# rwdavies/QUILT

Hardware: AMD Instinct MI355X
Metric: samples/sec on 2Mb region, K=50k haps, 1x coverage; dosage r2 vs CPU ref (higher is better)
Workload: dtype f64

## Files before the change

quilt_amd/csrc/gibbs.hip:

```cpp
#include "panel.hpp"

#include <chrono>
#include <functional>

#include <algorithm>
#include <cmath>
#include <cstdlib>
#include <map>
#include <memory>

#include "gibbs_dev.hpp"
#include "gibbs_blocks.hpp"

namespace qa {
int gibbs3_waves(int Ksp, int C, int share);
void launch_gibbs3(const void *gibbs_params, hipStream_t st);
void launch_block_rate3(const void *gibbs_params, hipStream_t st);
void launch_block3(const void *gibbs_params, hipStream_t st);
void launch_resample3(const void *gibbs_params, hipStream_t st);
}

namespace {

template <int NE, int NW>
__device__ void forward_full_both(Chain<NE, NW> &ch) {
    const int G = ch.G, Ksp = ch.Ksp;
    Col<NE> a[2], e[2];
    GridStreams<Chain<NE, NW>> gs;
    for (int g = 0; g < G; g++) {
        if ((g & 63) == 0) {
            if (g) gs.store_c(ch);
            gs.load_fwd(ch, g);
        }
        const int j = g & 63;
        ch.ld(e[0], ch.eg[0] + (size_t)g * Ksp);
        ch.ld(e[1], ch.eg[1] + (size_t)g * Ksp);
        const double s0 = rl_f64(gs.t0, j), s1 = rl_f64(gs.t1, j);
#pragma unroll
        for (int h = 0; h < 2; h++) {
#pragma unroll
            for (int i = 0; i < NE; i++) {
                if (g == 0) a[h].v[i] = ch.valid[i] ? ch.prior * e[h].v[i] : 0.0;
                else a[h].v[i] = ch.valid[i] ? e[h].v[i] * (s0 * a[h].v[i] + s1 * ch.prior) : 0.0;
            }
        }
        double sm[2];
        ch.sum_col2(a[0], a[1], sm[0], sm[1]);
        const double cc[2] = {1 / sm[0], 1 / sm[1]};
#pragma unroll
        for (int h = 0; h < 2; h++) {
#pragma unroll
            for (int i = 0; i < NE; i++) a[h].v[i] = a[h].v[i] * cc[h];
            ch.st(a[h], ch.alpha[h] + (size_t)g * Ksp);
        }
        gs.set_c(ch.lane, j, cc[0], cc[1]);
    }
    gs.store_c(ch);
    chain_sync<NW>();
}

template <int NE, int NW, bool FASTER>
__device__ void backward_both(Chain<NE, NW> &ch) {
    const int G = ch.G, Ksp = ch.Ksp;
    const double one_over_K = 1 / (double)ch.Ks;
    Col<NE> b[2], e[2];
    GridStreams<Chain<NE, NW>> gs;
    gs.load_bwd(ch, (G - 1) & ~63);
    {
        const int j = (G - 1) & 63;
        const double cl[2] = {rl_f64(gs.c0, j), rl_f64(gs.c1, j)};
#pragma unroll
        for (int h = 0; h < 2; h++) {
#pragma unroll
            for (int i = 0; i < NE; i++) b[h].v[i] = ch.valid[i] ? cl[h] : 0.0;
            ch.stm(b[h], ch.beta[h] + (size_t)(G - 1) * Ksp);
        }
    }
    if (G >= 2) {
        ch.ldm(e[0], ch.eg[0] + (size_t)(G - 1) * Ksp);
        ch.ldm(e[1], ch.eg[1] + (size_t)(G - 1) * Ksp);
    }
    for (int g = G - 2; g >= 0; --g) {
        if ((g & 63) == 63) gs.load_bwd(ch, g & ~63);
        const int j = g & 63;
        Col<NE> en[2];
        ch.ldm(en[0], ch.eg[0] + (size_t)g * Ksp);
        ch.ldm(en[1], ch.eg[1] + (size_t)g * Ksp);
        const double s0 = rl_f64(gs.t0, j), s1 = rl_f64(gs.t1, j);
        const double cg[2] = {rl_f64(gs.c0, j), rl_f64(gs.c1, j)};
        const bool has = !FASTER || rl_i32(gs.has, j) != 0;
        double x[2] = {0, 0};
#pragma unroll
        for (int h = 0; h < 2; h++) {
#pragma unroll
            for (int i = 0; i < NE; i++) {
                if (has) b[h].v[i] = e[h].v[i] * b[h].v[i];
                if (FASTER) x[h] += b[h].v[i];
                else x[h] += ch.valid[i] ? ch.prior * b[h].v[i] : 0.0;
            }
        }
        ch.template bsum<2>(x);
#pragma unroll
        for (int h = 0; h < 2; h++) {
            const double xx = FASTER ? s1 * x[h] * one_over_K : s1 * x[h];
#pragma unroll
            for (int i = 0; i < NE; i++) b[h].v[i] = ch.valid[i] ? cg[h] * (xx + s0 * b[h].v[i]) : 0.0;
            ch.stm(b[h], ch.beta[h] + (size_t)g * Ksp);
        }
        e[0] = en[0];
        e[1] = en[1];
    }
}

#ifndef QA_LEAN_WAVES
#define QA_LEAN_WAVES 2
#endif
template <int NE, int NW, bool LEAN>
__global__ __launch_bounds__(64 * NW) __attribute__((amdgpu_waves_per_eu(LEAN ? QA_LEAN_WAVES : 1))) void k_gibbs(GibbsParams p) {
    __shared__ double s_red[2 * NW * 4];
    __shared__ double s_e[LEAN ? 2 * NE * 64 * NW : 1];
    const int c = blockIdx.x, t = threadIdx.x;
    using CH = Chain<NE, NW>;
    CH ch(p, c, t, s_red);
    constexpr int NT = CH::NT;
    const int lane = ch.lane;
    const int G = ch.G, Ksp = ch.Ksp, R = ch.R, Ks = ch.Ks;
    const double prior = ch.prior;
    bool (&valid)[NE] = ch.valid;
    const double *runif = p.seed_reads ? nullptr : p.runif_reads + (size_t)p.read_off[c] * p.n_its;
    const uint64_t seed_reads = p.seed_reads ? p.seed_reads[c] : 0, seed_shard = p.seed_shard ? p.seed_shard[c] : 0;
    const int first_read = p.first_read[c];
    const bool init_iteratively = p.init_iteratively && first_read >= 0;

    for (int h = 0; h < 3; h++)
        for (int g = t; g < G; g += NT) ch.cv[h][g] = 0.0;
    for (int r = t; r < R; r += NT) ch.Hc[r] = 0;

    {
        Col<NE> one;
#pragma unroll
        for (int i = 0; i < NE; i++) one.v[i] = 1.0;
        for (int h = 0; h < 2; h++)
            for (int g = 0; g < G; g++) ch.st(one, ch.eg[h] + (size_t)g * Ksp);
    }
    chain_sync<NW>();
    if (!init_iteratively) {
        ReadStreams<CH> rs;
        rs.base = -1;
        int r = 0;
        while (r < R) {
            if ((r & 63) == 0 && rs.base != r) rs.load(ch, r, nullptr, 0);
            const int g = rl_i32(rs.wif, r & 63);
            Col<NE> e[2];
#pragma unroll
            for (int i = 0; i < NE; i++) e[0].v[i] = e[1].v[i] = 1.0;
            while (r < R) {
                if ((r & 63) == 0 && rs.base != r) rs.load(ch, r, nullptr, 0);
                if (rl_i32(rs.wif, r & 63) != g) break;
                Col<NE> er;
                {
                    typename CH::ErPre x;
                    ch.ld_pre(x, r);
                    ch.read_emission(er, x, rl_i32(rs.dn, r & 63));
                }
                const int h = rl_i32(rs.H, r & 63) - 1;
#pragma unroll
                for (int i = 0; i < NE; i++) {
                    if (h == 0) e[0].v[i] *= er.v[i];
                    else e[1].v[i] *= er.v[i];
                }
                r++;
            }
            ch.st(e[0], ch.eg[0] + (size_t)g * Ksp);
            ch.st(e[1], ch.eg[1] + (size_t)g * Ksp);
        }
        forward_full_both(ch);
        backward_both<NE, NW, false>(ch);
    } else {
        Col<NE> one;
#pragma unroll
        for (int i = 0; i < NE; i++) one.v[i] = valid[i] ? 1.0 : 0.0;
        for (int h = 0; h < 2; h++) {
            for (int g = 0; g < G; g++) {
                ch.st(one, ch.alpha[h] + (size_t)g * Ksp);
                ch.st(one, ch.beta[h] + (size_t)g * Ksp);
            }
            for (int g = t; g < G; g += NT) ch.cv[h][g] = 1.0;
        }
        chain_sync<NW>();
        for (int h = 0; h < 2; h++) {
            Col<NE> a;
#pragma unroll
            for (int i = 0; i < NE; i++) a.v[i] = valid[i] ? prior * 1.0 : 0.0;
            const double cc = 1 / ch.sum_col(a);
#pragma unroll
            for (int i = 0; i < NE; i++) a.v[i] = a.v[i] * cc;
            ch.st(a, ch.alpha[h]);
            if (t == 0) ch.cv[h][0] = cc;
        }
    }
    chain_sync<NW>();

    int shard_it = 0;
    int status = 0;
    for (int it = 0; it < p.n_its && status == 0; it++) {
        const bool last_sweep = it == p.n_its - 1;
        const bool steady = !init_iteratively || it >= 2;
        Col<NE> a[2];
        int iRead = 0;
        typename CH::ErPre pre_er;
        if (R > 0) ch.ld_pre(pre_er, 0);
        ReadStreams<CH> rs;
        rs.base = -1;
        GridStreams<CH> gs;
        Col<NE> e[2], bt[2];
        ch.ldm(e[0], ch.eg[0]);
        ch.ldm(e[1], ch.eg[1]);
        ch.ldm(bt[0], ch.beta[0]);
        ch.ldm(bt[1], ch.beta[1]);
        for (int g = 0; g < G; g++) {
            if ((g & 63) == 0) {
                if (g) gs.store_c(ch);
                gs.load_fwd(ch, g);
            }
            const int jg = g & 63;
            const bool has = rl_i32(gs.has, jg) != 0;
            Col<NE> en[LEAN ? 1 : 2], bn[LEAN ? 1 : 2];
            if constexpr (!LEAN) {
                const size_t gn = (size_t)min(g + 1, G - 1) * Ksp;
                ch.ldm(en[0], ch.eg[0] + gn);
                ch.ldm(en[1], ch.eg[1] + gn);
                ch.ldm(bn[0], ch.beta[0] + gn);
                ch.ldm(bn[1], ch.beta[1] + gn);
            }
            double cg[2];
            if (g > 0) {
                const double x = rl_f64(gs.t0, jg), t1 = rl_f64(gs.t1, jg);
                const double one_over_K = 1 / (double)Ks;
                const double c2v[2] = {rl_f64(gs.c0, jg), rl_f64(gs.c1, jg)};
                double sp[2];
                ch.sum_col2(a[0], a[1], sp[0], sp[1]);
#pragma unroll
                for (int h = 0; h < 2; h++) {
                    const double alphaConst = t1 * sp[h];
#pragma unroll
                    for (int i = 0; i < NE; i++) {
                        const double inner = (x * a[h].v[i] + alphaConst * one_over_K);
                        a[h].v[i] = valid[i] ? (has ? e[h].v[i] * inner : inner) : 0.0;
                    }
                }
                double sn[2];
                ch.sum_col2(a[0], a[1], sn[0], sn[1]);
#pragma unroll
                for (int h = 0; h < 2; h++) {
                    const double c2 = c2v[h];
                    double aa = 1 / (c2 * sn[h]);
                    cg[h] = c2 * aa;
                    aa *= c2;
#pragma unroll
                    for (int i = 0; i < NE; i++) a[h].v[i] *= aa;
                }
            } else {
#pragma unroll
                for (int h = 0; h < 2; h++) {
#pragma unroll
                    for (int i = 0; i < NE; i++) a[h].v[i] = valid[i] ? prior * e[h].v[i] : 0.0;
                }
                double sn[2];
                ch.sum_col2(a[0], a[1], sn[0], sn[1]);
#pragma unroll
                for (int h = 0; h < 2; h++) {
                    cg[h] = 1 / sn[h];
#pragma unroll
                    for (int i = 0; i < NE; i++) a[h].v[i] *= cg[h];
                }
            }
            bool changed = false;
            Col<NE> ab[2];
            double pC[2] = {1, 1};
            if (has) {
                double s[2] = {0, 0};
#pragma unroll
                for (int i = 0; i < NE; i++) {
                    ab[0].v[i] = a[0].v[i] * bt[0].v[i];
                    ab[1].v[i] = a[1].v[i] * bt[1].v[i];
                    s[0] += ab[0].v[i];
                    s[1] += ab[1].v[i];
                }
                ch.template bsum<2>(s);
// ... 85 lines not shown
                const double cs0 = p0, cs1 = p1 + p0;
                const int h_rN = (chance < cs0) ? 0 : ((chance < cs1) ? 1 : 0);
                if (((h_rN != h_rC) || ginit) && !pass) {
                    changed = true;
                    if (lane == jr) rs.H = h_rN + 1;
                    auto mul_e = [&](int h, const Col<NE> &f) {
                        if constexpr (LEAN) {
#pragma unroll
                            for (int i = 0; i < NE; i++) s_e[(h * NE + i) * NT + t] *= f.v[i];
                        } else {
#pragma unroll
                            for (int i = 0; i < NE; i++) e[h].v[i] *= f.v[i];
                        }
                    };
                    if (normal) {
                        if (h_rC == 0) {
#pragma unroll
                            for (int i = 0; i < NE; i++) { a[0].v[i] *= ri.v[i]; ab[0].v[i] *= ri.v[i]; }
                            mul_e(0, ri);
                        } else {
#pragma unroll
                            for (int i = 0; i < NE; i++) { a[1].v[i] *= ri.v[i]; ab[1].v[i] *= ri.v[i]; }
                            mul_e(1, ri);
                        }
                    }
                    if (h_rN == 0) {
#pragma unroll
                        for (int i = 0; i < NE; i++) { a[0].v[i] *= er.v[i]; ab[0].v[i] *= er.v[i]; }
                        mul_e(0, er);
                    } else {
#pragma unroll
                        for (int i = 0; i < NE; i++) { a[1].v[i] *= er.v[i]; ab[1].v[i] *= er.v[i]; }
                        mul_e(1, er);
                    }
                    if (normal || h_rN == 1) { pC[0] = pA1[0]; pC[1] = pA1[1]; }
                }
                if (last_sweep) {
                    const double x[3] = {p0, p1, 0.0};
                    const double rlc[7][3] = {{1, 0, 0}, {0, 1, 0}, {0, 0, 1}, {0.5 / (0.5 + 0.5), 0.5 / (0.5 + 0.5), 0},
                                              {0.5 / (0.5 + 0.0), 0, 0.0 / (0.5 + 0.0)},
                                              {0, 0.5 / (0.5 + 0.0), 0.0 / (0.5 + 0.0)}, {0.5, 0.5, 0.0}};
                    double local_min = 2;
                    int which = 8;
                    for (int i = 0; i < 7; i++) {
                        const double y = fabs(rlc[i][0] - x[0]) + fabs(rlc[i][1] - x[1]) + fabs(rlc[i][2] - x[2]);
                        if (y < local_min) { local_min = y; which = i; }
                    }
                    if (lane == jr) rs.Hc = (local_min < p.class_sum_cutoff) ? which + 1 : 0;
                }
            }
#ifndef QA_LEAN_LATE_E
            if constexpr (LEAN) {
                const size_t gn0 = (size_t)min(g + 1, G - 1) * Ksp;
                ch.ldm(e[0], ch.eg[0] + gn0);
                ch.ldm(e[1], ch.eg[1] + gn0);
            }
#endif
            if (changed) {
                double sm[2];
                ch.sum_col2(a[0], a[1], sm[0], sm[1]);
#pragma unroll
                for (int h = 0; h < 2; h++) {
                    const double alphaConst = 1 / sm[h];
                    cg[h] *= alphaConst;
#pragma unroll
                    for (int i = 0; i < NE; i++) a[h].v[i] = a[h].v[i] * alphaConst;
#ifndef QA_LEAN_LATE_E
                    if constexpr (LEAN) {
#pragma unroll
                        for (int i = 0; i < NE; i++) bt[h].v[i] = s_e[(h * NE + i) * NT + t];
                        ch.stm(bt[h], ch.eg[h] + (size_t)g * Ksp);
                    } else {
                        ch.stm(e[h], ch.eg[h] + (size_t)g * Ksp);
                    }
#else
                    if constexpr (LEAN) {
#pragma unroll
                        for (int i = 0; i < NE; i++) e[h].v[i] = s_e[(h * NE + i) * NT + t];
                    }
                    ch.stm(e[h], ch.eg[h] + (size_t)g * Ksp);
#endif
                }
            }
            if (last_sweep) {
#pragma unroll
                for (int h = 0; h < 2; h++) ch.stm(a[h], ch.alpha[h] + (size_t)g * Ksp);
            }
            gs.set_c(lane, jg, cg[0], cg[1]);
            if constexpr (LEAN) {
#ifndef QA_DBG_NO_LATE_LOADS
                const size_t gn = (size_t)min(g + 1, G - 1) * Ksp;
#ifdef QA_LEAN_LATE_E
                ch.ldm(e[0], ch.eg[0] + gn);
                ch.ldm(e[1], ch.eg[1] + gn);
#endif
                ch.ldm(bt[0], ch.beta[0] + gn);
                ch.ldm(bt[1], ch.beta[1] + gn);
#endif
            } else {
                e[0] = en[0]; e[1] = en[1];
                bt[0] = bn[0]; bt[1] = bn[1];
            }
        }
        gs.store_c(ch);
        if (rs.base >= 0) rs.store(ch);
        chain_sync<NW>();
#ifndef QA_DBG_SKIP_BWD
        backward_both<NE, NW, true>(ch);
#endif
        {
            double s[2] = {0, 0};
            for (int g = t; g < G; g += NT) { s[0] += ch.cv[0][g]; s[1] += ch.cv[1][g]; }
            ch.template bsum<2>(s);
            if (!isfinite(s[0]) || !isfinite(s[1])) status = 1;
        }
        if (p.per_it) {
            double s[4] = {0, 0, 0, 0};
            for (int g = t; g < G; g += NT) { s[0] -= log(ch.cv[0][g]); s[1] -= log(ch.cv[1][g]); }
            for (int r = t; r < R; r += NT) { const int h = ch.H[r]; s[2] += h == 1 ? 1.0 : 0.0; s[3] += h == 2 ? 1.0 : 0.0; }
            ch.template bsum<4>(s);
            if (t == 0) {
                double *o = p.per_it + ((size_t)c * p.n_its + it) * 8;
                o[0] = s[0]; o[1] = s[1]; o[2] = 0; o[3] = s[2]; o[4] = s[3]; o[5] = 0; o[6] = 0; o[7] = 0;
            }
        }
        if (status) break;
        bool to_block = false;
        for (int i = 0; i < p.n_block; i++) if (p.block_its[i] == it) to_block = true;
#ifdef QA_DBG_SKIP_SHARD
        to_block = false;
#endif
        if (to_block && p.do_shard) {
            const double *ru = p.runif_shard + ((size_t)c * p.n_block + shard_it) * (G - 1);
            shard_it++;
            double mloc1, mloc2, mlc1 = 0, mlc2 = 0;
            {
                double s[2] = {0, 0};
                for (int g = t; g < G; g += NT) { s[0] -= log(ch.cv[0][g]); s[1] -= log(ch.cv[1][g]); }
                ch.template bsum<2>(s);
                mloc1 = s[0]; mloc2 = s[1];
            }
            bool flip = false;
            int ir = 0;
            Col<NE> s_a[2];
            GridStreams<CH> ss;
            ReadStreams<CH> rr;
            rr.base = -1;
            bool rr_dirty = false;
            for (int g = 0; g < G; g++) {
                if ((g & 63) == 0) {
                    if (g) ss.store_c(ch);
                    ss.load_fwd(ch, g);
                }
                const int jg = g & 63;
                const double oc1 = rl_f64(ss.c0, jg), oc2 = rl_f64(ss.c1, jg);
                Col<NE> e2[2];
                ch.ldm(e2[0], ch.eg[flip ? 1 : 0] + (size_t)g * Ksp);
                ch.ldm(e2[1], ch.eg[flip ? 0 : 1] + (size_t)g * Ksp);
                Col<NE> b1, b2;
                if (!LEAN && g < G - 1) {
                    ch.ldm(b1, ch.beta[0] + (size_t)g * Ksp);
                    ch.ldm(b2, ch.beta[1] + (size_t)g * Ksp);
                }
                double cn[2];
                if (g == 0) {
#pragma unroll
                    for (int h = 0; h < 2; h++) {
#pragma unroll
                        for (int i = 0; i < NE; i++) s_a[h].v[i] = valid[i] ? prior * e2[h].v[i] : 0.0;
                    }
                    double sm[2];
                    ch.sum_col2(s_a[0], s_a[1], sm[0], sm[1]);
#pragma unroll
                    for (int h = 0; h < 2; h++) {
                        cn[h] = 1 / sm[h];
#pragma unroll
                        for (int i = 0; i < NE; i++) s_a[h].v[i] *= cn[h];
                    }
                } else {
                    if (flip) {
                        ch.stm(e2[0], ch.eg[0] + (size_t)g * Ksp);
                        ch.stm(e2[1], ch.eg[1] + (size_t)g * Ksp);
                    }
                    const double x = rl_f64(ss.t0, jg), t1 = rl_f64(ss.t1, jg);
                    double sp[2];
                    ch.sum_col2(s_a[0], s_a[1], sp[0], sp[1]);
#pragma unroll
                    for (int h = 0; h < 2; h++) {
                        const double alphaConst = t1 * sp[h];
                        const double c2 = (h == 0) ? oc1 : oc2;
#pragma unroll
                        for (int i = 0; i < NE; i++)
                            s_a[h].v[i] = valid[i] ? c2 * e2[h].v[i] * (x * s_a[h].v[i] + alphaConst * prior) : 0.0;
                    }
                    double sm[2];
                    ch.sum_col2(s_a[0], s_a[1], sm[0], sm[1]);
#pragma unroll
                    for (int h = 0; h < 2; h++) {
                        const double c2 = (h == 0) ? oc1 : oc2;
                        const double aa = 1 / sm[h];
                        cn[h] = c2 * aa;
#pragma unroll
                        for (int i = 0; i < NE; i++) s_a[h].v[i] *= aa;
                    }
                }
                if (last_sweep) {
                    ch.stm(s_a[0], ch.alpha[0] + (size_t)g * Ksp);
                    ch.stm(s_a[1], ch.alpha[1] + (size_t)g * Ksp);
                }
                ss.set_c(lane, jg, cn[0], cn[1]);
                mlc1 -= log(cn[0]);
                mlc2 -= log(cn[1]);
                while (ir < R) {
                    if ((ir & 63) == 0 && rr.base != ir) {
                        if (rr.base >= 0 && rr_dirty) rr.store(ch);
                        rr.load(ch, ir, nullptr, 0);
                        rr_dirty = false;
                    }
                    if (rl_i32(rr.wif, ir & 63) != g) break;
                    if (flip) {
                        if (lane == (ir & 63)) rr.H = 3 - rr.H;
                        rr_dirty = true;
                    }
                    ir++;
                }
                if (g < G - 1) {
                    if constexpr (LEAN) {
                        ch.ldm(b1, ch.beta[0] + (size_t)g * Ksp);
                        ch.ldm(b2, ch.beta[1] + (size_t)g * Ksp);
                    }
                    double s[4] = {0, 0, 0, 0};
#pragma unroll
                    for (int i = 0; i < NE; i++) {
                        s[0] += s_a[0].v[i] * b1.v[i];
                        s[1] += s_a[1].v[i] * b2.v[i];
                        s[2] += s_a[1].v[i] * b1.v[i];
                        s[3] += s_a[0].v[i] * b2.v[i];
                    }
                    ch.template bsum<4>(s);
                    const double pA1 = mlc1 + mloc1 + log(s[0]);
                    const double pA2 = mlc2 + mloc2 + log(s[1]);
                    const double pB1 = mlc2 + mloc1 + log(s[2]);
                    const double pB2 = mlc1 + mloc2 + log(s[3]);
                    const double diff = pB1 + pB2 - pA1 - pA2;
                    double probs1 = 1;
                    const double probs2 = exp(diff);
                    const double ps = probs1 + probs2;
                    probs1 /= ps;
                    const double ug = seed_shard ? stream_uniform(seed_shard, (uint64_t)(shard_it - 1) * (G - 1) + g) : ru[g];
                    flip = ug > probs1;
                }
                mloc1 += log(oc1);
                mloc2 += log(oc2);
            }
            ss.store_c(ch);
            if (rr.base >= 0 && rr_dirty) rr.store(ch);
            chain_sync<NW>();
            backward_both<NE, NW, false>(ch);
        }
    }
    if (t == 0) p.status[c] = status;
}

__global__ __launch_bounds__(256) void k_happrobs(GibbsParams p) {
    const int g = blockIdx.x, c = blockIdx.y;
    const int b = threadIdx.x & 31, part = threadIdx.x >> 5;
    __shared__ double s_g[3][8][32], s_t[3][8];
    extern __shared__ __attribute__((aligned(16))) char s_dyn[];
    const int Ks = p.Ks, Ksp = p.Ksp, G = p.G;
    double *const s_gk0 = reinterpret_cast<double *>(s_dyn);
    uint32_t *const s_w = reinterpret_cast<uint32_t *>(s_gk0 + (size_t)p.nH * Ksp);
    auto gk = [&](int h, int k) -> double & { return s_gk0[(size_t)h * Ksp + k]; };
    const int32_t *which = p.which + (size_t)c * Ks;
    const size_t mat = (size_t)G * Ksp;
    for (int k = threadIdx.x; k < Ks; k += 256) {
        const int kk = which[k];
        s_w[k] = panel_word(p, g, kk, p.hm[(size_t)g * p.Kp + kk]);
        for (int h = 0; h < p.nH; h++) {
            const size_t o = ((size_t)c * p.nH + h) * mat + (size_t)g * Ksp + k;
            const double x = 1 / p.cvec[((size_t)c * 3 + h) * G + g];
            gk(h, k) = (p.alpha[o] * p.beta[o]) * x;
        }
    }
    __syncthreads();
    const int s = 32 * g, nLocal = min(32, p.T - s);
    double acc[3] = {0, 0, 0}, tot[3] = {0, 0, 0};
    if (p.nH == 2) {
        for (int k = part; k < Ks; k += 8) {
            const bool on = (s_w[k] >> b) & 1u;
// ... 394 lines not shown
    GibbsLaunch(GibbsLaunch &&) = default;
    GibbsLaunch(const GibbsLaunch &) = delete;
};

GibbsLaunch launch_slice(const GibbsCall &a, const qa_gibbs_opts_t *o, const std::vector<size_t> &base_of, int G, int T, int c0, int c1) {
    GibbsLaunch L;
    L.c0 = c0; L.C = c1 - c0;
    const size_t chain0 = (size_t)c0, read0 = (size_t)a.read_off[c0], base0 = base_of[chain0];
    const size_t n_its = (size_t)(o->n_gibbs_burn_in_its + o->n_gibbs_sample_its), nb = (size_t)o->n_block_gibbs_iterations;
    auto from = [](auto *p, size_t off) { return p ? p + off : nullptr; };
    L.ff_chain = from(o->ff_chain, chain0);
    L.rep_id = from(o->reads_same_as, chain0);
    L.a.which = a.which + chain0 * o->Ks;
    L.a.first_read = a.first_read + chain0;
    L.a.underflow_problem = from(a.underflow_problem, chain0);
    L.a.seed_reads = from(a.seed_reads, chain0);
    L.a.seed_shard = from(a.seed_shard, chain0);
    L.a.hapProbs_t = from(a.hapProbs_t, chain0 * T * 3);
    L.a.genProbsM_t = from(a.genProbsM_t, chain0 * T * 3);
    L.a.genProbsF_t = from(a.genProbsF_t, chain0 * T * 3);
    L.a.state_out = a.state_out;
    L.read_off.resize((size_t)L.C + 1);
    for (int i = 0; i <= L.C; i++) L.read_off[(size_t)i] = a.read_off[c0 + i] - a.read_off[c0];
    L.a.read_off = L.read_off.data();
    L.a.read_ptr = a.read_ptr + read0 + chain0;
    L.a.wif = a.wif + read0;
    L.a.H = a.H + read0;
    L.a.H_class = from(a.H_class, read0);
    L.a.runif_reads = from(a.runif_reads, read0 * n_its);
    L.a.runif_shard = from(a.runif_shard, o->ff != 0.0 ? read0 * nb * 2 : chain0 * nb * (size_t)(G - 1));
    L.a.u = a.u + base0;
    L.a.bq = a.bq + base0;
    if (o->reads_same_as) {
        L.rep_off.resize((size_t)L.C);
        for (int c = c0; c < c1; c++) L.rep_off[(size_t)(c - c0)] = (int64_t)base_of[(size_t)o->reads_same_as[c]] - (int64_t)base0;
    }
    return L;
}

inline int32_t fold_base_quality(int32_t b, int32_t &last) {
    if (b == 0) b = last; else last = b;
    if (b > 255 || b < -255) throw std::runtime_error("|base quality| > 255");
    return b;
}

void fold_zero_base_qualities(const int32_t *rp, int R, int Jmax, int32_t *bq_eff_block) {
    int32_t last = 0;
    for (int r = 0; r < R; r++) {
        int J = rp[r + 1] - rp[r] - 1;
        if (J >= Jmax) J = Jmax;
        for (int j = 0; j <= J; j++) bq_eff_block[rp[r] + j] = fold_base_quality(bq_eff_block[rp[r] + j], last);
    }
}

std::vector<int32_t> checked_folded_qualities(int n, const int32_t *read_off, const int32_t *read_ptr, const int32_t *u, const int32_t *bq,
                                              const std::vector<int32_t> &base_off, int T, int Jmax) {
    std::vector<int32_t> bq_eff((size_t)std::max(base_off[n], 1));
    qa::parallel_for((size_t)n, qa::host_threads(), [&](size_t c) {
        const int R = read_off[c + 1] - read_off[c];
        const int32_t *rp = read_ptr + read_off[c] + c;
        const size_t b0 = (size_t)base_off[c];
        for (int i = 0; i < rp[R]; i++) {
            if (u[b0 + i] < 0 || u[b0 + i] >= T) throw std::runtime_error("read SNP index out of range");
            bq_eff[b0 + i] = bq[b0 + i];
        }
        fold_zero_base_qualities(rp, R, Jmax, bq_eff.data() + b0);
    });
    return bq_eff;
}

struct ChunkHost {
    int C, G, T, Ks, Ksp, NE, nH, n_its, nw, er_nt, er_padb, rc_words, totR, totB, maxR = 0;
    bool want_probs, want_pairs;
    bool aliased = false;
    size_t etot = 0, ixtot = 0;
    std::vector<int32_t> base_off, which0, bq_eff, dense_of, n_dense;
    std::vector<size_t> eoff, ixoff;
    std::vector<uint8_t> ghr;
    std::vector<uint32_t> rc_any;
    std::vector<int32_t> rep;
    std::vector<int64_t> hbase;
};

ChunkHost chunk_layout(qa_panel_t *pn, const qa_rare_common *rc, const qa_gibbs_opts_t *o, const GibbsLaunch &L) {
    ChunkHost h;
    const int C = h.C = L.C;
    h.G = rc ? rc->G_all : pn->G; h.T = rc ? rc->T_all : pn->T; h.Ks = o->Ks;
    h.Ksp = (h.Ks + 63) / 64 * 64; h.NE = h.Ksp / 64;
    h.nH = o->ff != 0.0 ? 3 : 2;
    h.rc_words = rc ? (h.T + 31) / 32 : 0;
    h.n_its = o->n_gibbs_burn_in_its + o->n_gibbs_sample_its;
    h.totR = L.a.read_off[C];
    h.want_probs = wants_probs(L.a, o);
    h.want_pairs = rc && h.want_probs && h.Ks <= 1024;
    h.nw = o->ff != 0.0 ? qa::gibbs3_waves(h.Ksp, C, pn->sharers()) : choose_gibbs_waves(h.Ksp, C, pn->exclusive ? 0 : pn->share);
    h.er_nt = 64 * h.nw; h.er_padb = padb_of(h.NE / h.nw);
    h.rc_any.assign((size_t)C * h.rc_words, 0u);
    h.base_off.assign(C + 1, 0); h.which0.resize((size_t)C * h.Ks);
    h.eoff.resize(C); h.ixoff.resize(C);
    h.ghr.assign((size_t)C * h.G, 0);
    h.dense_of.assign(std::max(h.totR, 1), -1);
    h.n_dense.assign(C, 0);
    for (int c = 0; c < C; c++) {
        const int R = L.a.read_off[c + 1] - L.a.read_off[c];
        h.maxR = std::max(h.maxR, R);
        const int32_t *rp = L.a.read_ptr + L.a.read_off[c] + c;
        h.base_off[c + 1] = h.base_off[c] + rp[R];
        h.ixoff[c] = h.ixtot;
        h.ixtot += (size_t)R * h.er_nt * h.er_padb;
    }
    h.totB = h.base_off[C];
    h.bq_eff.resize((size_t)std::max(h.totB, 1));
    return h;
}

void find_shared_reads(const GibbsLaunch &L, ChunkHost &h) {
    const int32_t *read_off = L.a.read_off, *read_ptr = L.a.read_ptr;
    const auto &base_off = h.base_off;
    h.rep.resize(h.C); h.hbase.resize(h.C);
    std::map<int32_t, int32_t> first_of;
    for (int c = 0; c < h.C; c++) {
        h.rep[c] = c;
        h.hbase[c] = L.rep_id ? L.rep_off[c] : (int64_t)base_off[c];
        if (!L.rep_id) continue;
        auto it = first_of.find(L.rep_id[c]);
        if (it == first_of.end()) { first_of.emplace(L.rep_id[c], c); h.aliased |= L.rep_off[c] != (int64_t)base_off[c]; continue; }
        const int r0 = it->second;
        const int R = read_off[c + 1] - read_off[c];
        if (read_off[r0 + 1] - read_off[r0] != R || base_off[r0 + 1] - base_off[r0] != base_off[c + 1] - base_off[c] ||
            std::memcmp(read_ptr + read_off[r0] + r0, read_ptr + read_off[c] + c, sizeof(int32_t) * ((size_t)R + 1)) != 0)
            throw std::runtime_error("reads_same_as names a chain with other reads");
        h.rep[c] = r0;
        h.aliased = true;
    }
}

void prepare_chain(const qa_panel_t *pn, const qa_rare_common *rc, const qa_gibbs_opts_t *o, const GibbsLaunch &L, ChunkHost &h, int c) {
    const int32_t *read_off = L.a.read_off, *wif = L.a.wif;
    const int G = h.G, T = h.T, Ks = h.Ks, rc_words = h.rc_words;
    const bool is_rep = h.rep[c] == c;
    const int R = read_off[c + 1] - read_off[c];
    const int32_t *rp = L.a.read_ptr + read_off[c] + c;
    const int64_t hb = h.hbase[c];
    int32_t *bq_eff = h.bq_eff.data() + (size_t)h.base_off[h.rep[c]];
    if (is_rep) std::memcpy(bq_eff, L.a.bq + hb, sizeof(int32_t) * (size_t)(h.base_off[c + 1] - h.base_off[c]));
    for (int r = 0; r < R; r++) {
        const int g = wif[read_off[c] + r];
        if (g < 0 || g >= G) throw std::runtime_error("read grid index out of range");
        if (r > 0 && g < wif[read_off[c] + r - 1]) throw std::runtime_error("reads must be sorted by grid");
        h.ghr[(size_t)c * G + g] = 1;
    }
    for (int k = 0; k < Ks; k++) {
        const int v = L.a.which[(size_t)c * Ks + k] - 1;
        if (v < 0 || v >= pn->K) throw std::runtime_error("which_haps_to_use out of range");
        h.which0[(size_t)c * Ks + k] = v;
        if (rc)
            for (int64_t i = rc->h_rare_ptr[v]; i < rc->h_rare_ptr[v + 1]; i++) {
                const int t = rc->h_rare_snp[i];
                h.rc_any[(size_t)c * rc_words + (t >> 5)] |= 1u << (t & 31);
            }
    }
    const int32_t *cu = L.a.u + hb;
    int32_t last = 0;
    int nd = 0;
    for (int r = 0; r < R; r++) {
        int J = rp[r + 1] - rp[r] - 1;
// ... 95 lines not shown
}

void upload_rare_pairs(qa::GibbsScratch &S, const qa_rare_common *rc, const ChunkHost &h, hipStream_t st) {
    const int C = h.C, G = h.G, Ks = h.Ks;
    std::vector<size_t> pbase((size_t)C + 1, 0);
    std::vector<std::vector<uint32_t>> keys((size_t)C);
    qa::parallel_for((size_t)C, qa::host_threads(), [&](size_t c) {
        auto &kv = keys[c];
        for (int k = 0; k < Ks; k++) {
            const int v = h.which0[c * Ks + k];
            for (int64_t i = rc->h_rare_ptr[v]; i < rc->h_rare_ptr[v + 1]; i++) kv.push_back(((uint32_t)rc->h_rare_snp[i] << 10) | (uint32_t)k);
        }
        std::sort(kv.begin(), kv.end());
    });
    for (int c = 0; c < C; c++) pbase[(size_t)c + 1] = pbase[(size_t)c] + keys[(size_t)c].size();
    std::vector<uint16_t> pairs(std::max<size_t>(pbase[(size_t)C], 1));
    std::vector<int32_t> poff((size_t)C * (G + 1), 0);
    for (int c = 0; c < C; c++) {
        const auto &kv = keys[(size_t)c];
        int32_t *po = poff.data() + (size_t)c * (G + 1);
        size_t i = 0;
        for (int g = 0; g < G; g++) {
            po[g] = (int32_t)i;
            while (i < kv.size() && (int)((kv[i] >> 10) >> 5) == g) {
                pairs[pbase[(size_t)c] + i] = (uint16_t)((((kv[i] >> 10) & 31u) << 10) | (kv[i] & 1023u));
                i++;
            }
        }
        po[G] = (int32_t)i;
    }
    S.rc_pairs.ensure(pairs.size()); S.rc_pairs.upload(pairs.data(), pairs.size(), st);
    S.rc_pair_off.ensure(poff.size()); S.rc_pair_off.upload(poff.data(), poff.size(), st);
    S.rc_pair_base.ensure((size_t)C); S.rc_pair_base.upload(pbase.data(), (size_t)C, st);
}

void carve_arena(qa::GibbsScratch &S, qa::Arena &arena, size_t arena_need, const ChunkHost &h) {
    const size_t mat = (size_t)h.C * h.nH * h.G * h.Ksp;
    S.er_idx.arena = S.er_tab.arena = &arena;
    S.eMatRead.arena = S.alpha.arena = S.beta.arena = S.eg.arena = S.cvec.arena = S.hap.arena = S.gm.arena = S.gf.arena = &arena;
    arena.require(arena_need);
    arena.reset();
    S.eMatRead.ensure(std::max<size_t>(h.etot, 1));
    S.er_idx.ensure(std::max<size_t>(h.ixtot, 1));
    S.er_tab.ensure(std::max<size_t>((size_t)h.totR * 64, 1));
    S.alpha.ensure(mat); S.beta.ensure(mat); S.eg.ensure(mat);
    S.cvec.ensure((size_t)h.C * 3 * h.G);
    if (h.want_probs) {
        S.hap.ensure((size_t)h.C * h.T * 3); S.gm.ensure((size_t)h.C * h.T * 3); S.gf.ensure((size_t)h.C * h.T * 3);
    }
}

GibbsParams fill_params(const qa::GibbsScratch &S, const qa_panel_t *pn, const qa_rare_common *rc, const qa_gibbs_opts_t *o,
                        const GibbsLaunch &L, const ChunkHost &h, hipStream_t st) {
    const int C = h.C;
    GibbsParams prm{};
    prm.hm = pn->hm.p; prm.B = pn->B.p; prm.sp_off = pn->sp_off.p; prm.sp_k = pn->sp_k.p;
    prm.sp_word = pn->sp_word.p; prm.sigma = S.tm.p; prm.Kp = pn->Kp; prm.G = h.G; prm.T = h.T;
    prm.nMaxDH = pn->nMaxDH; prm.ref_error = pn->ref_error;
    prm.C = C; prm.Ks = h.Ks; prm.Ksp = h.Ksp; prm.NE = h.NE; prm.which = S.which.p;
    prm.read_off = S.read_off.p; prm.read_ptr = S.read_ptr.p; prm.base_off = S.base_off.p;
    prm.u = S.u.p; prm.bq = S.bq.p; prm.wif = S.wif.p; prm.grid_has_read = S.ghr.p;
    prm.pR_tab = S.tabs.p; prm.pA_tab = S.tabs.p + 512;
    prm.Jmax = o->Jmax; prm.inv_maxdiff = 1 / o->maxDifferenceBetweenReads; prm.rescale = o->rescale_eMatRead_t;
    prm.n_its = h.n_its; prm.n_burn_in = o->n_gibbs_burn_in_its; prm.block_its = S.block_its.p;
    prm.n_block = o->perform_block_gibbs ? o->n_block_gibbs_iterations : 0;
    prm.do_shard = o->do_shard_block_gibbs; prm.init_iteratively = o->gibbs_initialize_iteratively;
    prm.disable_read_category_usage = o->disable_read_category_usage;
    prm.class_sum_cutoff = o->class_sum_cutoff;
    prm.nH = h.nH;
    prm.it_begin = 0; prm.it_end = h.n_its;
    prm.ff = o->ff;
    if (o->per_it_out) {
        QA_HIP(hipMemsetAsync(S.per_it.p, 0, sizeof(double) * C * h.n_its * 8, st));
        prm.per_it = S.per_it.p;
    }
    if (L.ff_chain) prm.ff_chain = S.ff_chain.p;
    prm.runif_reads = S.runif_reads.p; prm.first_read = S.first_read.p; prm.runif_shard = S.runif_shard.p;
    prm.seed_reads = L.a.seed_reads ? S.seeds.p : nullptr;
    prm.seed_shard = (L.a.seed_reads && L.a.seed_shard) ? S.seeds.p + C : nullptr;
    prm.eMatRead = S.eMatRead.p; prm.eread_off = S.eread_off.p; prm.is_cat1 = S.is_cat1.p; prm.er_nent = S.er_nent.p;
    prm.er_idx = S.er_idx.p; prm.eridx_off = S.eridx_off.p; prm.er_tab = S.er_tab.p; prm.dense_of = S.dense_of.p;
    prm.er_nt = h.er_nt; prm.er_padb = h.er_padb;
    prm.alpha = S.alpha.p; prm.beta = S.beta.p; prm.eg = S.eg.p; prm.cvec = S.cvec.p;
    prm.H = S.H.p; prm.H_class = S.H_class.p; prm.status = S.status.p;
    prm.hapProbs = S.hap.p; prm.genProbsM = S.gm.p; prm.genProbsF = S.gf.p;
    if (rc) {
        prm.rc_common = rc->common_index.p; prm.rc_rare_ptr = rc->rare_ptr.p; prm.rc_rare_snp = rc->rare_snp.p;
        prm.rc_any = S.rc_any.p; prm.rc_words = h.rc_words; prm.rc_Gc = pn->G;
        if (h.want_pairs) { prm.rc_pairs = S.rc_pairs.p; prm.rc_pair_off = S.rc_pair_off.p; prm.rc_pair_base = S.rc_pair_base.p; }
    }
    return prm;
}

void nipt_block_tables(const qa_gibbs_opts_t *o, const GibbsLaunch &L, const ChunkHost &h, const std::vector<double> &rate2,
                       const std::vector<int32_t> &seg_status, int n_thr, std::vector<int32_t> &h_where, std::vector<int32_t> &h_tab,
                       std::vector<int32_t> &h_n) {
    const int C = h.C, G = h.G;
    const int32_t *read_off = L.a.read_off;
    h_where.assign((size_t)C * G, -1); h_tab.assign((size_t)C * 4 * G, 0); h_n.assign(C, 0);
    qa::parallel_for((size_t)C, n_thr, [&](size_t c) {
        const int R = read_off[c + 1] - read_off[c];
        if (seg_status[c] != 0 || R < 1) return;
        const std::vector<int32_t> blocked = qa::define_blocked_grids(
            rate2.data() + c * G, o->L_grid, G, o->shuffle_bin_radius, o->block_gibbs_quantile_prob);
        const qa::BlockTable T = qa::make_gibbs_considers(blocked, L.a.wif + read_off[c], R);
        h_n[c] = T.n_blocks;
        std::copy(T.grid_where.begin(), T.grid_where.end(), h_where.begin() + c * G);
        int32_t *tb = h_tab.data() + c * 4 * G;
        for (int b = 0; b < T.n_blocks; b++) {
            tb[b] = T.grid_start[b]; tb[G + b] = T.grid_end[b];
            tb[2 * G + b] = T.reads_start[b]; tb[3 * G + b] = T.reads_end[b];
        }
    });
}

void nipt_sweeps(const GibbsParams &prm, qa::GibbsScratch &S, const qa_gibbs_opts_t *o, const GibbsLaunch &L, const ChunkHost &h,
                 hipStream_t st, bool tmg) {
    const int C = h.C, G = h.G, totR = h.totR, n_its = h.n_its;
    const int32_t *read_off = L.a.read_off;
    GibbsParams q = prm;
    q.ff = o->ff;
    const char *lean3_env = getenv("QA_GIBBS3_LEAN");
    const bool lean3_on = lean3_env && atoi(lean3_env) != 0;
    q.lean3 = (h.Ksp == 640 && h.nw == 1 && lean3_on) ? 1 : 0;
    q.blk_n_pass = std::max(o->n_block_gibbs_iterations, 1);
    std::vector<int> passes;
    if (o->perform_block_gibbs)
        for (int i = 0; i < o->n_block_gibbs_iterations; i++) {
            const int b = o->block_gibbs_iterations[i];
            if (b >= 0 && b < n_its && std::find(passes.begin(), passes.end(), b) == passes.end()) passes.push_back(b);
        }
    std::sort(passes.begin(), passes.end());
    if (!passes.empty()) {
        S.blk_rate2.ensure((size_t)C * G); S.blk_where.ensure((size_t)C * G);
        S.blk_tab.ensure((size_t)C * 4 * G); S.blk_n.ensure(C);
        q.blk_rate2 = S.blk_rate2.p; q.blk_where = S.blk_where.p; q.blk_tab = S.blk_tab.p; q.blk_n = S.blk_n.p;
    }
    std::vector<double> rate2;
    std::vector<int32_t> h_where, h_tab, h_n;
    int it0 = 0;
    q.rebuild = 0;
    for (size_t j = 0; j < passes.size(); j++) {
        q.it_begin = it0; q.it_end = passes[j] + 1;
        qa::launch_gibbs3(&q, st);
        q.rebuild = 1;
        qa::launch_block_rate3(&q, st);
        rate2.resize((size_t)C * G);
        S.blk_rate2.download(rate2.data(), rate2.size(), st);
        std::vector<int32_t> seg_status(C);
        S.status.download(seg_status.data(), C, st);
        QA_HIP(hipStreamSynchronize(st));
        const double tg0 = now_s();
        const int n_thr = std::max(1, std::min<int>(qa::host_threads(), C));
        nipt_block_tables(o, L, h, rate2, seg_status, n_thr, h_where, h_tab, h_n);
        const double tg1 = now_s();
        S.blk_where.upload(h_where.data(), h_where.size(), st);
        S.blk_tab.upload(h_tab.data(), h_tab.size(), st);
        S.blk_n.upload(h_n.data(), h_n.size(), st);
        q.blk_pass = (int)j;
        const bool draw_cb = o->draw_uniforms != nullptr;
        q.defer_resample = draw_cb ? 1 : 0;
        std::vector<double> ub;
        if (draw_cb) {
            for (int c = 0; c < C; c++) {
                const int R = read_off[c + 1] - read_off[c];
                if (R < 1) continue;
// ... 46 lines not shown
void download_probs(qa::GibbsScratch &S, const qa_gibbs_opts_t *o, const GibbsLaunch &L, const ChunkHost &h, hipStream_t st) {
    const GibbsCall &a = L.a;
    const int C = h.C, G = h.G, T = h.T;
    if (a.hapProbs_t) S.hap.download(a.hapProbs_t, (size_t)C * T * 3, st);
    if (o->hap_words_out) {
        int32_t *d_words = reinterpret_cast<int32_t *>(S.gm.p);
        hipLaunchKernelGGL(k_pack_hap_words, dim3((G + 255) / 256, 3, C), dim3(256), 0, st, S.hap.p, T, G, d_words);
        QA_HIP(hipGetLastError());
        if (a.genProbsM_t) throw std::runtime_error("hap_words_out cannot be combined with genProbs outputs");
        qa::staged_download(o->hap_words_out + (size_t)L.c0 * 3 * G, d_words, sizeof(int32_t) * (size_t)C * 3 * G, st);
    }
    if (o->hap_major_out) {
        const int nL = o->hap_major_labels;
        if (a.genProbsF_t || nL < 1 || nL > 3) throw std::runtime_error("hap_major_out: 1..3 labels, not combined with genProbs outputs");
        hipLaunchKernelGGL(k_hap_major, dim3((T + 255) / 256, C), dim3(256), 0, st, S.hap.p, T, nL, S.gf.p);
        QA_HIP(hipGetLastError());
        qa::staged_download(o->hap_major_out + (size_t)L.c0 * nL * T, S.gf.p, sizeof(double) * (size_t)C * nL * T, st);
    }
    if (a.genProbsM_t) S.gm.download(a.genProbsM_t, (size_t)C * T * 3, st);
    if (a.genProbsF_t) S.gf.download(a.genProbsF_t, (size_t)C * T * 3, st);
    QA_HIP(hipStreamSynchronize(st));
}

double profile_launch(hipEvent_t *ev, const ChunkHost &h, int n_block) {
    const int C = h.C, G = h.G, Ks = h.Ks, nH = h.nH, totR = h.totR, n_its = h.n_its;
    float ms[3];
    for (int i = 0; i < 3; i++) QA_HIP(hipEventElapsedTime(&ms[i], ev[i], ev[i + 1]));
    const double col = 2.0 * Ks * (double)G * 48.0;
    const double sweeps = (double)n_its * (C * col + (double)totR * Ks * 8.0) +
                          (1.0 + 2.0 * n_block) * C * col;
    const double t_e = qa::profile_clock_ms(ev[0]);
    const double passes = (double)n_its + 1.0 + 2.0 * n_block;
    const double units = (double)n_its * totR + passes * (double)C * G;
    const double serial = (double)n_its * h.maxR + passes * (double)G;
    qa::profile_add(qa::PK_EMATREAD, ms[0], (double)totR * Ks * 8.0, t_e);
    qa::profile_add(nH == 3 ? qa::PK_GIBBS3 : ((h.Ksp / 64 == 10 && h.nw == 1 && use_lean_build(C)) ? qa::PK_GIBBS_LEAN : qa::PK_GIBBS), ms[1],
                    sweeps * (nH / 2.0), t_e + ms[0], units, serial, (double)C);
    if (h.want_probs) qa::profile_add(qa::PK_HAPPROBS, ms[2], C * (double)nH * Ks * (double)G * 16.0, t_e + ms[0] + ms[1]);
    return ms[0] + ms[1] + ms[2];
}

void dump_state(const qa::GibbsScratch &S, const ChunkHost &h, double *state_out) {
    const int G = h.G, Ks = h.Ks, Ksp = h.Ksp;
    std::vector<double> tmp((size_t)G * Ksp);
    const qa::ABuf<double> *src[3] = {&S.alpha, &S.beta, &S.eg};
    size_t o2 = 0;
    for (int m = 0; m < 3; m++)
        for (int hl = 0; hl < 2; hl++) {
            QA_HIP(hipMemcpy(tmp.data(), src[m]->p + (size_t)hl * G * Ksp, sizeof(double) * tmp.size(),
                             hipMemcpyDeviceToHost));
            for (int g = 0; g < G; g++)
                for (int k = 0; k < Ks; k++) state_out[o2 + (size_t)g * Ks + k] = tmp[(size_t)g * Ksp + k];
            o2 += (size_t)G * Ks;
        }
    QA_HIP(hipMemcpy(state_out + o2, S.cvec.p, sizeof(double) * 3 * G, hipMemcpyDeviceToHost));
}

int gibbs_chunk(qa_panel_t *pn, size_t arena_need, const qa_rare_common *rc, const qa_gibbs_opts_t *o, const GibbsLaunch &L) {
    if (!g_gibbs) g_gibbs.reset(new GibbsHolder());
    auto &S = g_gibbs->s;
    const bool tmg = getenv("QA_TIMING") != nullptr;
    const double T0 = now_s();
    hipStream_t st = pn->gibbs_stream ? pn->gibbs_stream : pn->stream;
    ChunkHost h = chunk_layout(pn, rc, o, L);
    find_shared_reads(L, h);
    prepare_chains(pn, rc, o, L, h);
    const double T1 = now_s();
    upload_inputs(S, pn, rc, o, L, h, st);
    if (h.want_pairs) upload_rare_pairs(S, rc, h, st);
    const double hold_t0 = now_s();
    qa::GateHold hold;
    hold.acquire(pn->gate(), &pn->arena, h.C * h.nw, arena_need);
    const double T1g = now_s();
    carve_arena(S, hold.arena(), arena_need, h);
    const GibbsParams prm = fill_params(S, pn, rc, o, L, h, st);
    for (auto &e : g_gibbs->ev) if (!e) QA_HIP(hipEventCreate(&e));
    QA_HIP(hipStreamSynchronize(st));
    const double T2 = now_s();
    launch_gibbs(prm, h.maxR, st, g_gibbs->ev, h.want_probs, h.nw, [&] { nipt_sweeps(prm, S, o, L, h, st, tmg); });
    const std::vector<int32_t> status = download_labels(S, o, L, h, st);
    const double T3 = now_s();
    hold.mark();
    download_probs(S, o, L, h, st);
    const bool dump = L.a.state_out && h.C == 1;
    if (!dump) hold.release();
    const double kernel_ms = profile_launch(g_gibbs->ev, h, prm.n_block);
    if (tmg)
        fprintf(stderr, "[qa_gibbs C=%d] host prep %.3f s, tables+uploads %.3f s (of which queued for the device %.3f s), kernels %.3f s (events %.3f), downloads %.3f s\n", h.C,
                T1 - T0, T2 - T1, T1g - hold_t0, T3 - T2, kernel_ms / 1e3, now_s() - T3);
    int ret = QA_OK;
    for (int c = 0; c < h.C; c++) {
        if (L.a.underflow_problem) L.a.underflow_problem[c] = status[c];
        if (status[c]) ret = QA_UNDERFLOW;
    }
    if (dump) dump_state(S, h, L.a.state_out);
    return ret;
}

int gibbs_batch_impl(qa_panel_t *pn, const qa_rare_common *rc, const qa_gibbs_opts_t *o, int32_t n_chain, const GibbsCall &a) {
    if (!qa::device_ready()) return QA_ERR_NO_DEVICE;
    if (!pn || !o || n_chain <= 0 || !a.which || !a.read_off || !a.read_ptr || !a.u || !a.bq || !a.wif ||
        (!a.runif_reads && !a.seed_reads) || !a.first_read || !a.H) {
        qa::set_error("qa_gibbs_batch: null argument");
        return QA_ERR_INVALID;
    }
    if ((o->ff != 0.0) != (o->sample_is_diploid == 0) || o->ff < 0 || o->ff >= 1) {
        qa::set_error("qa_gibbs_batch: ff > 0 goes with sample_is_diploid = 0 (NIPT), ff = 0 with sample_is_diploid = 1");
        return QA_ERR_INVALID;
    }
    if (o->ff != 0.0 && o->perform_block_gibbs && o->n_block_gibbs_iterations > 0 &&
        (!o->L_grid || o->shuffle_bin_radius <= 0 || !(o->block_gibbs_quantile_prob > 0 && o->block_gibbs_quantile_prob < 1) ||
         (!a.runif_shard && !a.seed_shard && !a.seed_reads && !o->draw_uniforms))) {
        qa::set_error("qa_gibbs_batch: the NIPT block Gibbs needs opts->L_grid, shuffle_bin_radius, block_gibbs_quantile_prob "
                      "and the block passes' uniforms (runif_shard, seeds, or opts->draw_uniforms)");
        return QA_ERR_INVALID;
    }
    if (o->draw_uniforms && (o->ff == 0.0 || a.seed_reads || a.seed_shard)) {
        qa::set_error("qa_gibbs_batch: opts->draw_uniforms serves the NIPT block passes (ff > 0) of a call with explicit uniforms "
                      "(runif_reads given, no seeds)");
        return QA_ERR_INVALID;
    }
    if (a.seed_shard && !a.seed_reads) {
        qa::set_error("qa_gibbs_batch: seed_shard goes with seed_reads (the two counter-based streams of a chain)");
        return QA_ERR_INVALID;
    }
    {
        const bool passes = o->perform_block_gibbs && o->n_block_gibbs_iterations > 0 && (o->ff != 0.0 || o->do_shard_block_gibbs);
        if (passes && !a.runif_shard && !(a.seed_reads && a.seed_shard) && !(o->ff != 0.0 && o->draw_uniforms)) {
            qa::set_error("qa_gibbs_batch: block / shard passes requested without their uniforms (runif_shard, or seed_reads and "
                          "seed_shard)");
            return QA_ERR_INVALID;
        }
    }
    if (o->ff_chain) {
        bool ok = o->ff != 0.0;
        for (int c = 0; c < n_chain && ok; c++) ok = o->ff_chain[c] > 0 && o->ff_chain[c] < 1;
        if (!ok) {
            qa::set_error("qa_gibbs_batch: ff_chain goes with ff > 0 (NIPT) and holds fetal fractions in (0, 1)");
            return QA_ERR_INVALID;
        }
    }
    const int32_t *read_off = a.read_off, *read_ptr = a.read_ptr;
    if (o->reads_same_as)
        for (int c = 0; c < n_chain; c++) {
            const int r0 = o->reads_same_as[c];
            if (r0 < 0 || r0 > c || o->reads_same_as[r0] != r0 || read_off[r0 + 1] - read_off[r0] != read_off[c + 1] - read_off[c]) {
                qa::set_error("qa_gibbs_batch: reads_same_as[%d] must name an earlier chain (or the chain itself) that names itself and has as many reads", c);
                return QA_ERR_INVALID;
            }
        }
    if (o->Ks <= 0 || o->Ks > QA_KSUBSET_MAX) {
        qa::set_error("qa_gibbs_batch: Ksubset = %d outside 1..%d", o->Ks, QA_KSUBSET_MAX);
        return QA_ERR_UNSUPPORTED;
    }
    if (o->ff != 0.0 && o->Ks > QA_KSUBSET_MAX_NIPT) {
        qa::set_error("qa_gibbs_batch: Ksubset = %d is not built for the NIPT sampler (ff > 0), which runs every Ksubset in 1..%d; "
                      "the diploid sampler runs 1..%d", o->Ks, QA_KSUBSET_MAX_NIPT, QA_KSUBSET_MAX);
        return QA_ERR_UNSUPPORTED;
    }
    return qa::guarded([&] {
        QA_HIP(hipSetDevice(pn->device));
        const int G = rc ? rc->G_all : pn->G, T = rc ? rc->T_all : pn->T, Ks = o->Ks, Ksp = (Ks + 63) / 64 * 64;
        const bool want_probs = wants_probs(a, o);
        std::vector<size_t> base_of(n_chain + 1, 0);
        for (int c = 0; c < n_chain; c++) {
            const int R = read_off[c + 1] - read_off[c];
            base_of[c + 1] = base_of[c] + (size_t)(read_ptr + read_off[c] + c)[R];
// ... 319 lines not shown
```

quilt_amd/csrc/gibbs_dev.hpp:

```cpp
#pragma once

#include "panel.hpp"

#include <cstdint>

namespace {

struct GibbsParams {
    const uint8_t *hm;
    const int32_t *B;
    const int32_t *sp_off;
    const int32_t *sp_k;
    const uint32_t *sp_word;
    const double *sigma;
    int Kp, G, T, nMaxDH;
    double ref_error;
    int C;
    int Ks, Ksp, NE;
    const int32_t *which;
    const int32_t *read_off;
    const int32_t *read_ptr;
    const int32_t *base_off;
    const int32_t *u;
    const int32_t *bq;
    const int32_t *wif;
    const uint8_t *grid_has_read;
    const double *pR_tab, *pA_tab;
    int Jmax;
    double inv_maxdiff;
    int rescale;
    int n_its, n_burn_in;
    const int32_t *block_its;
    int n_block;
    int do_shard;
    int init_iteratively;
    int nH;
    int disable_read_category_usage;
    double class_sum_cutoff;
    const double *runif_reads;
    const int32_t *first_read;
    const double *runif_shard;
    const uint64_t *seed_reads, *seed_shard;
    double *eMatRead;
    const size_t *eread_off;
    uint8_t *er_idx;
    const size_t *eridx_off;
    double *er_tab;
    const int32_t *dense_of;
    int er_nt, er_padb;
    uint8_t *is_cat1;
    uint8_t *er_nent;
    double *alpha, *beta, *eg;
    double *cvec;
    int32_t *H;
    int32_t *H_class;
    int32_t *status;
    double *hapProbs, *genProbsM, *genProbsF;
    const int32_t *rc_common;
    const int64_t *rc_rare_ptr;
    const int32_t *rc_rare_snp;
    const uint32_t *rc_any;
    int rc_words, rc_Gc;
    const int32_t *rc_pair_off;
    const size_t *rc_pair_base;
    const uint16_t *rc_pairs;
    int it_begin, it_end;
    int rebuild;
    int lean3;
    const int32_t *blk_where;
    const int32_t *blk_tab;
    const int32_t *blk_n;
    double *blk_rate2;
    int blk_pass, blk_n_pass;
    int defer_resample;
    double ff;
    const double *ff_chain;
    double *per_it;
};

__device__ __forceinline__ bool rare_has_alt(const GibbsParams &p, int hap, int snp) {
    int64_t lo = p.rc_rare_ptr[hap], hi = p.rc_rare_ptr[hap + 1];
    while (lo < hi) {
        const int64_t mid = (lo + hi) >> 1;
        const int v = p.rc_rare_snp[mid];
        if (v == snp) return true;
        if (v < snp) lo = mid + 1; else hi = mid;
    }
    return false;
}

template <int CTRL, int ROW_MASK>
__device__ __forceinline__ double dpp_get(double v) {
    int lo = __double2loint(v), hi = __double2hiint(v);
    lo = __builtin_amdgcn_update_dpp(0, lo, CTRL, ROW_MASK, 0xf, true);
    hi = __builtin_amdgcn_update_dpp(0, hi, CTRL, ROW_MASK, 0xf, true);
    return __hiloint2double(hi, lo);
}
__device__ __forceinline__ double wsum(double v) {
    v += dpp_get<0x111, 0xf>(v);
    v += dpp_get<0x112, 0xf>(v);
    v += dpp_get<0x114, 0xf>(v);
    v += dpp_get<0x118, 0xf>(v);
    v += dpp_get<0x142, 0xa>(v);
    v += dpp_get<0x143, 0xc>(v);
    const int lo = __builtin_amdgcn_readlane(__double2loint(v), 63);
    const int hi = __builtin_amdgcn_readlane(__double2hiint(v), 63);
    return __hiloint2double(hi, lo);
}
__device__ __forceinline__ void wsum2(double &a, double &b) {
    const auto lo = __builtin_amdgcn_permlane32_swap(__double2loint(a), __double2loint(b), false, false);
    const auto hi = __builtin_amdgcn_permlane32_swap(__double2hiint(a), __double2hiint(b), false, false);
    double v = __hiloint2double(hi[0], lo[0]) + __hiloint2double(hi[1], lo[1]);
    v += dpp_get<0x111, 0xf>(v);
    v += dpp_get<0x112, 0xf>(v);
    v += dpp_get<0x114, 0xf>(v);
    v += dpp_get<0x118, 0xf>(v);
    v += dpp_get<0x142, 0xa>(v);
    a = __hiloint2double(__builtin_amdgcn_readlane(__double2hiint(v), 31), __builtin_amdgcn_readlane(__double2loint(v), 31));
    b = __hiloint2double(__builtin_amdgcn_readlane(__double2hiint(v), 63), __builtin_amdgcn_readlane(__double2loint(v), 63));
}
__device__ __forceinline__ double fold32(double a, double b) {
    const auto lo = __builtin_amdgcn_permlane32_swap(__double2loint(a), __double2loint(b), false, false);
    const auto hi = __builtin_amdgcn_permlane32_swap(__double2hiint(a), __double2hiint(b), false, false);
    return __hiloint2double(hi[0], lo[0]) + __hiloint2double(hi[1], lo[1]);
}
__device__ __forceinline__ double fold16_rows(double ab, double cd) {
    const auto lo = __builtin_amdgcn_permlane16_swap(__double2loint(ab), __double2loint(cd), false, false);
    const auto hi = __builtin_amdgcn_permlane16_swap(__double2hiint(ab), __double2hiint(cd), false, false);
    double v = __hiloint2double(hi[0], lo[0]) + __hiloint2double(hi[1], lo[1]);
    v += dpp_get<0x111, 0xf>(v);
    v += dpp_get<0x112, 0xf>(v);
    v += dpp_get<0x114, 0xf>(v);
    v += dpp_get<0x118, 0xf>(v);
    return v;
}
__device__ __forceinline__ double lane_of(double v, int l) {
// ... 493 lines not shown
```

Before: 37.41.

## Fuse read-emission build into initial forward pass and skip unneeded alpha stores

Merges the initial per-grid read emission construction into the forward pass, so emissions are computed and consumed in one sweep instead of being written, then reloaded. Drops the separate fill of eg with ones in the non-iterative path. Alpha stores in the init forward and the last sweep are now gated on whether probabilities or state output are actually requested, which saves memory traffic when they are not. This assumes the grid points without reads get their eg filled by the fused loop, and it adds a new param flag.

```diff
diff --git a/quilt_amd/csrc/gibbs.hip b/quilt_amd/csrc/gibbs.hip
--- a/quilt_amd/csrc/gibbs.hip
+++ b/quilt_amd/csrc/gibbs.hip
@@ -23,18 +23,42 @@
 namespace {
 
 template <int NE, int NW>
-__device__ void forward_full_both(Chain<NE, NW> &ch) {
-    const int G = ch.G, Ksp = ch.Ksp;
-    Col<NE> a[2], e[2];
-    GridStreams<Chain<NE, NW>> gs;
+__device__ void build_forward_both(Chain<NE, NW> &ch, bool store_alpha) {
+    using CH = Chain<NE, NW>;
+    const int G = ch.G, Ksp = ch.Ksp, R = ch.R;
+    Col<NE> a[2];
+    GridStreams<CH> gs;
+    ReadStreams<CH> rs;
+    rs.base = -1;
+    int r = 0;
     for (int g = 0; g < G; g++) {
         if ((g & 63) == 0) {
             if (g) gs.store_c(ch);
             gs.load_fwd(ch, g);
         }
         const int j = g & 63;
-        ch.ld(e[0], ch.eg[0] + (size_t)g * Ksp);
-        ch.ld(e[1], ch.eg[1] + (size_t)g * Ksp);
+        Col<NE> e[2];
+#pragma unroll
+        for (int i = 0; i < NE; i++) e[0].v[i] = e[1].v[i] = 1.0;
+        while (r < R) {
+            if ((r & 63) == 0 && rs.base != r) rs.load(ch, r, nullptr, 0);
+            if (rl_i32(rs.wif, r & 63) != g) break;
+            Col<NE> er;
+            {
+                typename CH::ErPre x;
+                ch.ld_pre(x, r);
+                ch.read_emission(er, x, rl_i32(rs.dn, r & 63));
+            }
+            const int h = rl_i32(rs.H, r & 63) - 1;
+#pragma unroll
+            for (int i = 0; i < NE; i++) {
+                if (h == 0) e[0].v[i] *= er.v[i];
+                else e[1].v[i] *= er.v[i];
+            }
+            r++;
+        }
+        ch.stm(e[0], ch.eg[0] + (size_t)g * Ksp);
+        ch.stm(e[1], ch.eg[1] + (size_t)g * Ksp);
         const double s0 = rl_f64(gs.t0, j), s1 = rl_f64(gs.t1, j);
 #pragma unroll
         for (int h = 0; h < 2; h++) {
@@ -51,7 +75,7 @@
         for (int h = 0; h < 2; h++) {
 #pragma unroll
             for (int i = 0; i < NE; i++) a[h].v[i] = a[h].v[i] * cc[h];
-            ch.st(a[h], ch.alpha[h] + (size_t)g * Ksp);
+            if (store_alpha) ch.stm(a[h], ch.alpha[h] + (size_t)g * Ksp);
         }
         gs.set_c(ch.lane, j, cc[0], cc[1]);
     }
@@ -136,45 +160,9 @@
         for (int g = t; g < G; g += NT) ch.cv[h][g] = 0.0;
     for (int r = t; r < R; r += NT) ch.Hc[r] = 0;
 
-    {
-        Col<NE> one;
-#pragma unroll
-        for (int i = 0; i < NE; i++) one.v[i] = 1.0;
-        for (int h = 0; h < 2; h++)
-            for (int g = 0; g < G; g++) ch.st(one, ch.eg[h] + (size_t)g * Ksp);
-    }
     chain_sync<NW>();
     if (!init_iteratively) {
-        ReadStreams<CH> rs;
-        rs.base = -1;
-        int r = 0;
-        while (r < R) {
-            if ((r & 63) == 0 && rs.base != r) rs.load(ch, r, nullptr, 0);
-            const int g = rl_i32(rs.wif, r & 63);
-            Col<NE> e[2];
-#pragma unroll
-            for (int i = 0; i < NE; i++) e[0].v[i] = e[1].v[i] = 1.0;
-            while (r < R) {
-                if ((r & 63) == 0 && rs.base != r) rs.load(ch, r, nullptr, 0);
-                if (rl_i32(rs.wif, r & 63) != g) break;
-                Col<NE> er;
-                {
-                    typename CH::ErPre x;
-                    ch.ld_pre(x, r);
-                    ch.read_emission(er, x, rl_i32(rs.dn, r & 63));
-                }
-                const int h = rl_i32(rs.H, r & 63) - 1;
-#pragma unroll
-                for (int i = 0; i < NE; i++) {
-                    if (h == 0) e[0].v[i] *= er.v[i];
-                    else e[1].v[i] *= er.v[i];
-                }
-                r++;
-            }
-            ch.st(e[0], ch.eg[0] + (size_t)g * Ksp);
-            ch.st(e[1], ch.eg[1] + (size_t)g * Ksp);
-        }
-        forward_full_both(ch);
+        build_forward_both(ch, p.n_its == 0 && p.alpha_out);
         backward_both<NE, NW, false>(ch);
     } else {
         Col<NE> one;
@@ -182,6 +170,7 @@
         for (int i = 0; i < NE; i++) one.v[i] = valid[i] ? 1.0 : 0.0;
         for (int h = 0; h < 2; h++) {
             for (int g = 0; g < G; g++) {
+                ch.stm(one, ch.eg[h] + (size_t)g * Ksp);
                 ch.st(one, ch.alpha[h] + (size_t)g * Ksp);
                 ch.st(one, ch.beta[h] + (size_t)g * Ksp);
             }
@@ -205,6 +194,7 @@
     int status = 0;
     for (int it = 0; it < p.n_its && status == 0; it++) {
         const bool last_sweep = it == p.n_its - 1;
+        const bool store_alpha = last_sweep && p.alpha_out;
         const bool steady = !init_iteratively || it >= 2;
         Col<NE> a[2];
         int iRead = 0;
@@ -456,7 +446,7 @@
 #endif
                 }
             }
-            if (last_sweep) {
+            if (store_alpha) {
 #pragma unroll
                 for (int h = 0; h < 2; h++) ch.stm(a[h], ch.alpha[h] + (size_t)g * Ksp);
             }
@@ -578,7 +568,7 @@
                         for (int i = 0; i < NE; i++) s_a[h].v[i] *= aa;
                     }
                 }
-                if (last_sweep) {
+                if (store_alpha) {
                     ch.stm(s_a[0], ch.alpha[0] + (size_t)g * Ksp);
                     ch.stm(s_a[1], ch.alpha[1] + (size_t)g * Ksp);
                 }
@@ -1139,6 +1129,8 @@
     std::vector<int64_t> hbase;
 };
 
+bool wants_state(const GibbsLaunch &L, const ChunkHost &h) { return L.a.state_out && h.C == 1; }
+
 ChunkHost chunk_layout(qa_panel_t *pn, const qa_rare_common *rc, const qa_gibbs_opts_t *o, const GibbsLaunch &L) {
     ChunkHost h;
     const int C = h.C = L.C;
@@ -1400,6 +1392,7 @@
     prm.er_idx = S.er_idx.p; prm.eridx_off = S.eridx_off.p; prm.er_tab = S.er_tab.p; prm.dense_of = S.dense_of.p;
     prm.er_nt = h.er_nt; prm.er_padb = h.er_padb;
     prm.alpha = S.alpha.p; prm.beta = S.beta.p; prm.eg = S.eg.p; prm.cvec = S.cvec.p;
+    prm.alpha_out = h.want_probs || wants_state(L, h);
     prm.H = S.H.p; prm.H_class = S.H_class.p; prm.status = S.status.p;
     prm.hapProbs = S.hap.p; prm.genProbsM = S.gm.p; prm.genProbsF = S.gf.p;
     if (rc) {
@@ -1612,7 +1605,7 @@
     const double T3 = now_s();
     hold.mark();
     download_probs(S, o, L, h, st);
-    const bool dump = L.a.state_out && h.C == 1;
+    const bool dump = wants_state(L, h);
     if (!dump) hold.release();
     const double kernel_ms = profile_launch(g_gibbs->ev, h, prm.n_block);
     if (tmg)
diff --git a/quilt_amd/csrc/gibbs_dev.hpp b/quilt_amd/csrc/gibbs_dev.hpp
--- a/quilt_amd/csrc/gibbs_dev.hpp
+++ b/quilt_amd/csrc/gibbs_dev.hpp
@@ -52,6 +52,7 @@
     uint8_t *er_nent;
     double *alpha, *beta, *eg;
     double *cvec;
+    int alpha_out;
     int32_t *H;
     int32_t *H_class;
     int32_t *status;
```

Result: slower. 36.94 (-1.3%).
